# togheppi/pytorch-super-resolution-model-collection

Measured on AMD Instinct MI355X. Metric: ESPCN x4 LR->HR images/sec (infer), higher is better.
Workload: dtype f32 storage/accumulate; fp32-faithful products on the fp16 matrix cores: operands scaled by exact powers of two, split into two fp16 planes, 3 MFMAs per product (f16x3, ~3e-7 rms vs fp64, like fp32 MFMA); 1 GPU; c2: ESPCN x4 inference, 256x256 LR, batch 64 per GPU, fp32, random-init N(0,0.02); parallelism=replicas x1 (no collective)

## Files before the change

pytorch_super_resolution_model_collection_amd/csrc/conv_pair.hip:

```cpp
#include "conv_bfw.h"

namespace srk {

namespace {

constexpr int PR_TH = 8, PR_TW = 16, PR_HW = 18;
constexpr int PR_NSLOTPIX = 6 * PR_HW, PR_NPIXP = PR_NSLOTPIX + 2;
constexpr int PR_NKEEP = 2 * PR_HW, PR_KP = PR_NKEEP + 2;
constexpr int PR_XR = 14, PR_XC = 23, PR_XP = 24;
constexpr int PR_NSLOT = 3, PR_NKBUF = 3;
constexpr int PR_WL2 = 9 * 2 * 256;
constexpr int PR_HBUF = 4 * PR_NPIXP;
constexpr int PR_KBUF = 2 * 4 * PR_KP;
constexpr int PR_PLANE = PR_NSLOT * PR_HBUF + PR_NKBUF * PR_KBUF;
constexpr int PR_XPQ = PR_XR * PR_XP * 16;
constexpr int PR_XT = PR_XPQ + 32;
constexpr int PR_XBUF = PR_XT + PR_XR * PR_XP * 8;
constexpr unsigned long long PR_FPIX = 0xfdb9eca875316420ull;
constexpr unsigned PR_AMAX_CAP = 1u << 14;
constexpr int PR_ARRIVE = 1, PR_DEPART = 2;
constexpr int PR_XLD = 24;
constexpr int PR_W1P = 2 * 2 * 8 * 64;
constexpr int PR_W1P_FLOATS = 144;
constexpr size_t PR_W1P_BYTES = (size_t)PR_W1P * 16 + PR_W1P_FLOATS * 4;
constexpr size_t PR_LDS = (size_t)PR_WL2 * 16 + (size_t)2 * PR_PLANE * 16 + (size_t)2 * PR_XBUF + 64;
static_assert(PR_LDS <= 160 * 1024, "k_espcn_pair: LDS");

__device__ unsigned g_pair_timeouts = 0;
__device__ unsigned g_pair_scans = 0;

typedef unsigned v4u_t __attribute__((ext_vector_type(4)));

struct PairParams {
  const float* x;
  const uint4* w1p;
  const float* b1;
  const uint4* wq2;
  const float* w2_descale;
  const float* b2;
  float* y;
  float* x_amax;
  float* y_amax;
  size_t xn;
  int amax_mode;
  int N, H, W, OH, OW, tiles_y, img_tiles, ntiles;
  unsigned x_img_bytes, y_bytes;
};

__device__ __forceinline__ float pr_slice_absmax(const float* __restrict__ x, size_t lo, size_t hi, size_t n, bool tail,
                                                 int t, int nt) {
  const f32x4* x4 = reinterpret_cast<const f32x4*>(x);
  float m = 0.f;
  for (size_t base = lo; base < hi; base += (size_t)nt * PR_XLD) {
    f32x4 v[PR_XLD];
#pragma unroll
    for (int k = 0; k < PR_XLD; ++k) {
      const size_t e = base + (size_t)t + (size_t)k * nt;
      v[k] = x4[e < hi ? e : hi - 1];
    }
#pragma unroll
    for (int k = 0; k < PR_XLD; ++k) m = abs_max4(m, v[k]);
  }
  if (tail) {
    const size_t e = (n & ~(size_t)3) + (size_t)t;
    if (t < 3 && e < n) m = fmaxf(m, fabsf(x[e]));
  }
  return m;
}

enum { PR_KTAP, PR_KROW, PR_KNONE };
struct PrKGroup {
  int kind, dy, dx;
};
__device__ __forceinline__ constexpr PrKGroup pr_kgroup(int ks, int kq) {
  if (ks < 5) return {PR_KTAP, ks, kq};
  if (ks == 5) return {PR_KTAP, (kq >> 1) + 2 * (kq & 1), 4};
  if (ks == 6) return kq == 0 ? PrKGroup{PR_KTAP, 4, 4} : (kq == 1 ? PrKGroup{PR_KNONE, 0, 0} : PrKGroup{PR_KROW, 2 * kq - 4, 0});
  return kq == 3 ? PrKGroup{PR_KNONE, 0, 0} : PrKGroup{PR_KROW, kq == 2 ? 4 : 2 * kq + 1, 0};
}

__global__ __launch_bounds__(128) void k_espcn_pair_prep(const float* __restrict__ w1, const float* __restrict__ b1,
                                                         uint4* __restrict__ out) {
  const int lane = threadIdx.x & 63, c1 = threadIdx.x >> 6;
  const int j = lane & 15, kq = lane >> 4;
  float wsum = 0.f, wmax = 0.f;
  {
    const float* wc = w1 + lane * 75;
    for (int i = 0; i < 75; ++i) {
      const float a = fabsf(wc[i]);
      wsum += a;
      wmax = fmaxf(wmax, a);
    }
  }
  const float wm = wave_max(wmax);
  const float sw1 = exp2i(amax_scale_exp(wm));
#pragma unroll
  for (int nf = 0; nf < 2; ++nf) {
    const int co = c1 * 32 + nf * 16 + j;
#pragma unroll
    for (int ks = 0; ks < 8; ++ks) {
      const PrKGroup g = pr_kgroup(ks, kq);
      float f[8];
#pragma unroll
      for (int e = 0; e < 8; ++e) {
        const bool tap = g.kind == PR_KTAP;
        const bool on = tap || (g.kind == PR_KROW && e < 5);
        const int ci = tap ? (e < 6 ? e % 3 : e - 6) : 2, dx = tap ? g.dx : (e < 5 ? e : 0);
        f[e] = on ? w1[((co * 3 + ci) * 5 + g.dy) * 5 + dx] : 0.f;
      }
      uint4 pl[2];
      split8h(f, sw1, pl);
      out[((c1 * 2 + nf) * 8 + ks) * 64 + lane] = g.kind == PR_KTAP ? make_uint4(pl[0].x, pl[0].y, pl[0].z, pl[1].w) : pl[1];
    }
  }
  if (c1 == 0) {
    float* t = reinterpret_cast<float*>(out + PR_W1P);
    t[lane] = wsum;
    t[64 + lane] = fabsf(b1[lane]);
    if (lane == 0) t[128] = wm;
  }
}

__global__ __launch_bounds__(512, 1) void k_espcn_pair(PairParams B) {
  extern __shared__ __attribute__((aligned(16))) uint4 smem4[];
  uint4* wl2 = smem4;
  uint4* ring = smem4 + PR_WL2;
  uint4* keep = ring + PR_NSLOT * PR_HBUF;
  unsigned char* xin_all = reinterpret_cast<unsigned char*>(ring + 2 * PR_PLANE);
  lds_cnt_t* cnt = (lds_cnt_t*)(xin_all + 2 * PR_XBUF);
  const int tid = threadIdx.x, lane = tid & 63, wave = tid >> 6;
  const int grp = wave >> 2, gw = wave & 3, lt = tid & 255;
  const int j = lane & 15, kq = lane >> 4;
  unsigned char* xin = xin_all + grp * PR_XBUF;

  const float* w1t = reinterpret_cast<const float*>(B.w1p + PR_W1P);
  const int nblk = gridDim.x;
  float xmax = 0.f;
  if (tid < 14) cnt[tid] = 0u;
  if (B.amax_mode) {
    float* red = reinterpret_cast<float*>(xin_all);
    const size_t n4 = B.xn >> 2;
    const float m = wave_max(pr_slice_absmax(B.x, (size_t)blockIdx.x * n4 / nblk, (size_t)(blockIdx.x + 1) * n4 / nblk, B.xn,
                                             blockIdx.x == 0, tid, 512));
    if (lane == 0) red[wave] = m;
    __syncthreads();
    if (tid == 0) {
      float b = red[0];
#pragma unroll
      for (int i = 1; i < 8; ++i) b = fmaxf(b, red[i]);
      const unsigned was = atomicMax(reinterpret_cast<unsigned*>(B.x_amax + (blockIdx.x & 15) * 16), __float_as_uint(b));
      asm volatile("s_waitcnt vmcnt(0)" ::"v"(was) : "memory");
      __hip_atomic_fetch_add(reinterpret_cast<unsigned*>(B.x_amax) + PR_ARRIVE, 1u, __ATOMIC_RELAXED, __HIP_MEMORY_SCOPE_AGENT);
    }
  } else {
    xmax = amax_read(B.x_amax);
  }

  {
    static_assert(PR_WL2 == 9 * 512, "k_espcn_pair: filter copy");
    v4u_t wv[9];
#pragma unroll
    for (int i = 0; i < 9; ++i) wv[i] = *reinterpret_cast<const v4u_t*>(B.wq2 + tid + 512 * i);
#pragma unroll
    for (int i = 0; i < 9; ++i) *reinterpret_cast<v4u_t*>(wl2 + tid + 512 * i) = wv[i];
  }

  const int c1 = gw >> 1, mh = gw & 1;
  const int mhu = __builtin_amdgcn_readfirstlane(mh), rhu = __builtin_amdgcn_readfirstlane(gw >> 1);
  uint4 w1f[2][8];
#pragma unroll
  for (int nf = 0; nf < 2; ++nf)
#pragma unroll
    for (int ks = 0; ks < 8; ++ks) w1f[nf][ks] = B.w1p[((c1 * 2 + nf) * 8 + ks) * 64 + lane];
  const float wsum = w1t[lane], babs = w1t[64 + lane];
  const int jp = (int)((PR_FPIX >> (4 * j)) & 15);
  int mpix[5], moff[5], tpix[2], toff[2];
#pragma unroll
  for (int m = 0; m < 5; ++m) {
    mpix[m] = 16 * (m < 4 ? 4 * mh + m : 8) + jp;
    const int p = PR_NKEEP + mpix[m];
    moff[m] = (p / PR_HW) * PR_XP + p % PR_HW + kq;
  }
#pragma unroll
  for (int m = 0; m < 2; ++m) {
    tpix[m] = 16 * (2 * mh + m) + jp;
    const int p = tpix[m] < PR_NKEEP ? tpix[m] : PR_NKEEP - 1;
    toff[m] = (p / PR_HW) * PR_XP + p % PR_HW + kq;
  }
  const int k5 = pr_kgroup(5, kq).dy * PR_XP + 4 - kq;
  int kmul[2], kadd[2], kd[2];
#pragma unroll
  for (int s = 0; s < 2; ++s) {
    const PrKGroup own = pr_kgroup(6 + s, kq), g = own.kind == PR_KNONE ? pr_kgroup(6 + s, kq - 1) : own;
    kmul[s] = g.kind == PR_KTAP ? 16 : 8;
    kd[s] = g.kind == PR_KTAP ? 8 : 32;
    asm volatile("" : "+v"(kd[s]));
    kadd[s] = g.kind == PR_KTAP ? 16 * (g.dy * PR_XP + g.dx - kq) : PR_XT + 8 * (g.dy * PR_XP - kq);
  }
  const int wr_slot = (kq >> 1) * PR_NPIXP * 16 + (kq & 1) * 8, wr_keep = (c1 * 4 + (kq >> 1)) * PR_KP * 16 + (kq & 1) * 8;

  const int rh = gw >> 1, nf2 = gw & 1;
  const int pj = j < 4 ? 2 * j : (j < 12 ? 2 * j - 7 : 2 * j - 16);
  const int lane_b = (4 * rh - 2) * PR_HW + pj + kq * PR_NPIXP;
  const int lane_k = pj + kq * PR_KP;
  const int lane_a = kq * 32 + nf2 * 16 + j;
  float b2v[4];
#pragma unroll
  for (int e = 0; e < 4; ++e) b2v[e] = B.b2[nf2 * 16 + 4 * kq + e];

  const int xcd = blockIdx.x & 7;
  int first, count;
  {
    const int lb = xcd * (nblk >> 3) + (xcd < (nblk & 7) ? xcd : (nblk & 7)) + (blockIdx.x >> 3);
    const int per = B.ntiles / nblk, rem = B.ntiles - per * nblk;
    first = lb * per + (lb < rem ? lb : rem);
    count = per + (lb < rem ? 1 : 0);
  }
  count = __builtin_amdgcn_readfirstlane(count);

  const __amdgpu_buffer_rsrc_t yr = buffer_rsrc(B.y, B.y_bytes);
  const unsigned HW_ = (unsigned)(B.H * B.W);
  float xv[2][3];
  auto xload = [&](int i) {
    const bool valid = i < count;
    const int t = first + (valid ? i : 0);
    const int n = t / B.img_tiles, rem = t - n * B.img_tiles;
    const int tx = rem / B.tiles_y, ty = rem - tx * B.tiles_y;
    const __amdgpu_buffer_rsrc_t xr = buffer_rsrc(B.x + (size_t)n * 3 * HW_, B.x_img_bytes);
#pragma unroll
    for (int s = 0; s < 2; ++s) {
      const int q = lt + 256 * s, qy = q / PR_XC, qx = q - qy * PR_XC;
      const bool ok = valid && q < PR_XR * PR_XC;
      const unsigned o = ok ? 4u * (unsigned)((ty * PR_TH + qy) * B.W + tx * PR_TW + qx) : 0x80000000u;
#pragma unroll
      for (int c = 0; c < 3; ++c)
        xv[s][c] = __builtin_bit_cast(float, __builtin_amdgcn_raw_buffer_load_b32(xr, (int)(o + (ok ? 4u * c * HW_ : 0u)), 0, 0));
    }
  };
  auto l1_frags = [&](auto nm, const int* off, f32x4 (*a)[2]) {
    constexpr int NM = decltype(nm)::value;
#pragma unroll
    for (int m = 0; m < NM; ++m) a[m][0] = a[m][1] = (f32x4){0.f, 0.f, 0.f, 0.f};
#pragma unroll
    for (int ks = 0; ks < 8; ++ks) {
#pragma unroll
      for (int m = 0; m < NM; ++m) {
        uint4 xc;
        if (ks < 6) {
          xc = *reinterpret_cast<const uint4*>(xin + 16 * (off[m] + (ks < 5 ? ks * PR_XP : k5)));
        } else {
          const int pa = __mul24(off[m], kmul[ks & 1]) + kadd[ks & 1];
          const uint2 ca = *reinterpret_cast<const uint2*>(xin + pa), cb = *reinterpret_cast<const uint2*>(xin + pa + kd[ks & 1]);
          xc = make_uint4(ca.x, ca.y, cb.x, cb.y);
        }
#pragma unroll
        for (int nf = 0; nf < 2; ++nf) a[m][nf] = mfma16h(w1f[nf][ks], xc, a[m][nf]);
      }
    }
  };
  bool dead = false;
  float amax = 0.f;
  xload(grp);
  if (B.amax_mode && wave == 0) {
    unsigned* ctr = reinterpret_cast<unsigned*>(B.x_amax);
    bool late = B.amax_mode == 2;
    if (!late) {
      unsigned spins = 0;
      while ((int)((unsigned)__builtin_amdgcn_readfirstlane((int)__hip_atomic_load(ctr + PR_ARRIVE, __ATOMIC_RELAXED,
                                                                                   __HIP_MEMORY_SCOPE_AGENT)) -
                   (unsigned)nblk) < 0) {
        __builtin_amdgcn_s_sleep(16);
        if (++spins > PR_AMAX_CAP) {
          late = true;
          break;
        }
      }
    }
    asm volatile("" ::: "memory");
    const float sv = wave_max(__hip_atomic_load(B.x_amax + (lane & 15) * 16, __ATOMIC_RELAXED, __HIP_MEMORY_SCOPE_AGENT));
    if (lane == 0) {
      cnt[14] = __float_as_uint(sv);
      cnt[15] = late ? 1u : 0u;
      const unsigned d = __hip_atomic_fetch_add(ctr + PR_DEPART, 1u, __ATOMIC_RELAXED, __HIP_MEMORY_SCOPE_AGENT);
      if (d + 1u == (unsigned)nblk) {
        __hip_atomic_store(ctr + PR_ARRIVE, 0u, __ATOMIC_RELAXED, __HIP_MEMORY_SCOPE_AGENT);
        __hip_atomic_store(ctr + PR_DEPART, 0u, __ATOMIC_RELAXED, __HIP_MEMORY_SCOPE_AGENT);
      }
    }
  }
  __syncthreads();
  if (B.amax_mode) {
    xmax = __uint_as_float(lds_cnt_peek(cnt + 14));
    if (lds_cnt_peek(cnt + 15)) {
      float* red = reinterpret_cast<float*>(xin_all);
      const float m = wave_max(pr_slice_absmax(B.x, 0, B.xn >> 2, B.xn, true, tid, 512));
      if (lane == 0) red[wave] = m;
      __syncthreads();
#pragma unroll
      for (int i = 0; i < 8; ++i) xmax = fmaxf(xmax, red[i]);
      xmax = __uint_as_float((unsigned)__builtin_amdgcn_readfirstlane((int)__float_as_uint(xmax)));
      __syncthreads();
      if (tid == 0) atomicAdd(&g_pair_scans, 1u);
    }
  }
  for (int i = tid; i < 2 * PR_XBUF / 16; i += 512) reinterpret_cast<uint4*>(xin_all)[i] = make_uint4(0u, 0u, 0u, 0u);
  __syncthreads();
  const int kx = amax_scale_exp(xmax);
  const float bnd = wave_max(fabsf(babs) + wsum * xmax);
  const int kw1 = amax_scale_exp(w1t[128]);
  const int km = amax_scale_exp(bnd);
  const float sx1 = exp2i(kx), sxm = exp2i(km);
  const float dsc1 = exp2i(-kx) * exp2i(-kw1);
  const float dsc2 = exp2i(-km) * B.w2_descale[0];

  unsigned own = 0;
  unsigned kseq = 0;
  int typrev = 0;
  for (int i = grp; i < count; i += 2, ++own) {
    const int t = first + i;
    const int n = t / B.img_tiles, rem = t - n * B.img_tiles;
    const int tx = rem / B.tiles_y, ty = rem - tx * B.tiles_y;
    const bool fresh = i == 0 || ty == 0;
    const bool hand = i + 1 < count && ty + 1 < B.tiles_y;
    kseq = i == grp ? (grp == 0 ? 1u : 2u + (ty == 0 ? 1u : 0u))
                    : kseq + 2u + (typrev + 1 == B.tiles_y ? 1u : 0u) + (ty == 0 ? 1u : 0u);
    typrev = ty;
    const unsigned kb = kseq % PR_NKBUF, ku = kseq / PR_NKBUF, tb = (kseq - 1u) % PR_NKBUF, tu = (kseq - 1u) / PR_NKBUF;
#pragma unroll
    for (int s = 0; s < 2; ++s) {
      const int q = lt + 256 * s;
      if (q < PR_XR * PR_XC) {
        const int qy = q / PR_XC, qx = q - qy * PR_XC;
        unsigned h01, m01, h2, m2;
        split2h(xv[s][0], xv[s][1], sx1, h01, m01);
        split2h(xv[s][2], 0.f, sx1, h2, m2);
        *reinterpret_cast<uint4*>(xin + 16 * (qy * PR_XP + qx)) = make_uint4(h01, h2 | (m01 << 16), (m01 >> 16) | (m2 << 16), h01);
        unsigned short* tq = reinterpret_cast<unsigned short*>(xin + PR_XT) + 4 * (qy * PR_XP + qx);
#pragma unroll
        for (int k = 0; k < 4; ++k) tq[-3 * k] = (unsigned short)h2;
      }
    }
    lds_cnt_signal(cnt + 6 + grp);
    xload(i + 2);
    lds_cnt_wait(cnt + 6 + grp, 4u * (own + 1), dead);

    float b1v[2][4];
#pragma unroll
    for (int nf = 0; nf < 2; ++nf)
#pragma unroll
      for (int e = 0; e < 4; ++e) b1v[nf][e] = B.b1[c1 * 32 + nf * 16 + 4 * kq + e];
    auto l1_store = [&](const f32x4 (&a)[2], unsigned char* base, int pix, int pitch) {
#pragma unroll
      for (int nf = 0; nf < 2; ++nf) {
        float v[4];
#pragma unroll
        for (int e = 0; e < 4; ++e) v[e] = fmaxf(__builtin_fmaf(a[nf][e], dsc1, b1v[nf][e]), 0.f);
        unsigned h01, m01, h23, m23;
        split2h(v[0], v[1], sxm, h01, m01);
        split2h(v[2], v[3], sxm, h23, m23);
        *reinterpret_cast<uint2*>(base + ((2 * nf) * pitch + pix) * 16) = make_uint2(h01, h23);
        *reinterpret_cast<uint2*>(base + (PR_PLANE + (2 * nf) * pitch + pix) * 16) = make_uint2(m01, m23);
      }
    };
    auto l1_tile = [&](auto nm) {
      constexpr int NM = decltype(nm)::value;
      f32x4 a1[NM][2];
      l1_frags(nm, moff, a1);
      const unsigned st = 2u * (unsigned)i + c1, slot = st % PR_NSLOT, use = st / PR_NSLOT;
      unsigned char* hb = reinterpret_cast<unsigned char*>(ring + slot * PR_HBUF) + wr_slot;
      lds_cnt_wait(cnt + 3 + slot, 4u * use, dead);
#pragma unroll
      for (int m = 0; m < NM; ++m)
        if (mpix[m] < PR_NSLOTPIX) l1_store(a1[m], hb, mpix[m], PR_NPIXP);
      lds_cnt_signal(cnt + slot);
      unsigned char* kp = reinterpret_cast<unsigned char*>(keep + kb * PR_KBUF) + wr_keep;
      lds_cnt_wait(cnt + 11 + kb, 8u * ku, dead);
#pragma unroll
      for (int m = 2; m < NM; ++m)
        if (mpix[m] >= PR_NSLOTPIX) l1_store(a1[m], kp, mpix[m] - PR_NSLOTPIX, PR_KP);
      lds_cnt_signal(cnt + 8 + kb);
    };
    const int vr = B.OH - ty * PR_TH;
    if (mhu == 1 && vr <= 3) {
      const unsigned st = 2u * (unsigned)i + c1, slot = st % PR_NSLOT, use = st / PR_NSLOT;
      lds_cnt_wait(cnt + 3 + slot, 4u * use, dead);
      lds_cnt_signal(cnt + slot);
      lds_cnt_wait(cnt + 11 + kb, 8u * ku, dead);
      lds_cnt_signal(cnt + 8 + kb);
    } else if (mh == (int)(own & 1)) {
      l1_tile(std::integral_constant<int, 5>{});
    } else {
      l1_tile(std::integral_constant<int, 4>{});
    }
    if (fresh) {
      f32x4 at[2][2];
      l1_frags(std::integral_constant<int, 2>{}, toff, at);
      unsigned char* kp = reinterpret_cast<unsigned char*>(keep + tb * PR_KBUF) + wr_keep;
      lds_cnt_wait(cnt + 11 + tb, 8u * tu, dead);
#pragma unroll
      for (int m = 0; m < 2; ++m)
        if (tpix[m] < PR_NKEEP) l1_store(at[m], kp, tpix[m], PR_KP);
      lds_cnt_signal(cnt + 8 + tb);
    }

    lds_cnt_wait(cnt + 8 + (rh == 0 ? tb : kb), 4u * ((rh == 0 ? tu : ku) + 1u), dead);
    if (rhu == 1 && vr <= 4) {
#pragma unroll
      for (int cc = 0; cc < 2; ++cc) {
        const unsigned st = 2u * (unsigned)i + cc, slot = st % PR_NSLOT, use = st / PR_NSLOT;
        lds_cnt_wait(cnt + slot, 2u * (use + 1), dead);
        lds_cnt_signal(cnt + 3 + slot);
      }
      lds_cnt_signal(cnt + 11 + tb, fresh ? 2u : 1u);
      lds_cnt_signal(cnt + 11 + kb, hand ? 1u : 2u);
    } else {
      f32x4 acc[4];
#pragma unroll
      for (int r = 0; r < 4; ++r) acc[r] = (f32x4){0.f, 0.f, 0.f, 0.f};
#pragma unroll
      for (int cc = 0; cc < 2; ++cc) {
        const unsigned st = 2u * (unsigned)i + cc, slot = st % PR_NSLOT, use = st / PR_NSLOT;
        lds_cnt_wait(cnt + slot, 2u * (use + 1), dead);
        const uint4* hb = ring + slot * PR_HBUF + lane_b;
        const uint4* kr = keep + (rh == 0 ? tb : kb) * PR_KBUF + cc * 4 * PR_KP + lane_k - (rh == 0 ? 0 : 4 * PR_HW);
        const uint4* pa = rh == 0 ? kr : hb;
        const uint4* pc = rh == 0 ? hb : kr;
#pragma unroll
        for (int v = 0; v < 3; ++v) {
          uint4 fa[3][2];
#pragma unroll
          for (int u = 0; u < 3; ++u) {
            fa[u][0] = wl2[((u * 3 + v) * 2 + cc) * 256 + lane_a];
            fa[u][1] = wl2[((u * 3 + v) * 2 + cc) * 256 + 128 + lane_a];
          }
#pragma unroll
          for (int R = 0; R < 6; ++R) {
            const uint4* px = R < 2 ? pa : (R < 4 ? hb : pc);
            const uint4 xh = px[R * PR_HW + v], xm = px[R * PR_HW + v + PR_PLANE];
#pragma unroll
            for (int u = 0; u < 3; ++u) {
              const int r = R - u;
              if (r >= 0 && r < 4) {
                acc[r] = mfma16h(fa[u][0], xm, acc[r]);
                acc[r] = mfma16h(fa[u][1], xh, acc[r]);
                acc[r] = mfma16h(fa[u][0], xh, acc[r]);
              }
            }
          }
        }
        lds_cnt_signal(cnt + 3 + slot);
      }
      lds_cnt_signal(cnt + 11 + tb, fresh ? 2u : 1u);
      lds_cnt_signal(cnt + 11 + kb, hand ? 1u : 2u);
      const int oc = tx * PR_TW + pj;
#pragma unroll
      for (int r = 0; r < 4; ++r) {
        const int orow = ty * PR_TH + 4 * rh + r;
        const bool ok = oc < B.OW && orow < B.OH;
        f32x4 v;
#pragma unroll
        for (int e = 0; e < 4; ++e) v[e] = fmaxf(__builtin_fmaf(acc[r][e], dsc2, b2v[e]), 0.f);
        if (ok) amax = fmaxf(amax, fmaxf(fmaxf(v[0], v[1]), fmaxf(v[2], v[3])));
        const unsigned o = ok ? 4u * (unsigned)(((n * B.OH + orow) * B.OW + oc) * 32 + nf2 * 16 + 4 * kq) : 0x80000000u;
        __builtin_amdgcn_raw_buffer_store_b128(__builtin_bit_cast(v4u_t, v), yr, (int)o, 0, 0);
      }
    }
  }
  if (B.y_amax) amax_commit(B.y_amax, amax, blockIdx.x + wave, amax_peek(B.y_amax, blockIdx.x + wave));
  if (dead && lane == 0) atomicAdd(&g_pair_timeouts, 1u);
}

}

int espcn_pair_launch(int N, int H, int W, const float* x, const void* w1p, const float* b1, const void* wp2,
                      const float* b2, float* y, float* x_amax, int amax_mode, float* y_amax, bool force, hipStream_t s) {
  if (N < 1 || H < 7 || W < 7 || !x_amax) return -1;
  const int OH = H - 6, OW = W - 6;
  const int tiles_y = (OH + PR_TH - 1) / PR_TH, tiles_x = (OW + PR_TW - 1) / PR_TW;
  const long ntiles = (long)N * tiles_y * tiles_x;
  const size_t x_img = (size_t)3 * H * W * 4, y_bytes = (size_t)N * OH * OW * 32 * 4;
  if (ntiles >= (1L << 29) || x_img >= (1ull << 31) || y_bytes >= (1ull << 31)) return -1;
  if (!force) {
    if ((double)OH * OW < 0.85 * (double)tiles_y * tiles_x * (PR_TH * PR_TW)) return -1;
    if (ntiles < 4L * kNumCU) return -1;
  }
  const size_t elems = (size_t)9 * 64 * 32;
  const char* prepared = reinterpret_cast<const char*>(wp2) + bf3_prepared_offset(elems);
  const char* fsec = prepared + f16_section_offset(64, 32, 9);
  PairParams B{};
  B.x = x; B.w1p = reinterpret_cast<const uint4*>(w1p); B.b1 = b1; B.b2 = b2; B.y = y; B.x_amax = x_amax; B.y_amax = y_amax;
  B.xn = (size_t)N * 3 * H * W;
  B.amax_mode = amax_mode;
  B.wq2 = reinterpret_cast<const uint4*>(fsec);
  B.w2_descale = reinterpret_cast<const float*>(fsec + bf3_main_bytes(64, 32, 9));
  B.N = N; B.H = H; B.W = W; B.OH = OH; B.OW = OW; B.tiles_y = tiles_y; B.img_tiles = tiles_x * tiles_y;
  B.ntiles = (int)ntiles;
  B.x_img_bytes = (unsigned)x_img;
  B.y_bytes = (unsigned)y_bytes;
  int grid = kNumCU;
  if (grid > ntiles) grid = (int)ntiles;
  note_amax_written(y_amax != nullptr);
  note_kernel("k_espcn_pair");
  launch_lds<&k_espcn_pair>(dim3(grid), dim3(512), PR_LDS, s, B);
  return check_launch("espcn_pair");
}

int pair_ring_timeouts(int reset) {
  unsigned v = 0;
  if (hipMemcpyFromSymbol(&v, HIP_SYMBOL(g_pair_timeouts), sizeof(v)) != hipSuccess) {
    (void)hipGetLastError();
    return -1;
  }
  if (reset && v) {
    const unsigned z = 0;
    (void)hipMemcpyToSymbol(HIP_SYMBOL(g_pair_timeouts), &z, sizeof(z));
  }
  return (int)v;
}

int pair_scans(int reset) {
  unsigned v = 0;
  if (hipMemcpyFromSymbol(&v, HIP_SYMBOL(g_pair_scans), sizeof(v)) != hipSuccess) {
    (void)hipGetLastError();
    return -1;
  }
  if (reset && v) {
    const unsigned z = 0;
    (void)hipMemcpyToSymbol(HIP_SYMBOL(g_pair_scans), &z, sizeof(z));
  }
  return (int)v;
}

int espcn_pair_prepare(const float* w1, const float* b1, void* out, hipStream_t s) {
  hipLaunchKernelGGL(k_espcn_pair_prep, dim3(1), dim3(128), 0, s, w1, b1, reinterpret_cast<uint4*>(out));
  return check_launch("espcn_pair_prepare");
}
size_t espcn_pair_prepared_bytes() { return PR_W1P_BYTES; }

}

extern "C" size_t srk_espcn_pair_prepared_bytes(void) { return srk::espcn_pair_prepared_bytes(); }

extern "C" int srk_espcn_pair_prepare(const float* w1, const float* b1, void* w1_prepared, void* stream) {
  SRK_REQUIRE(w1 && b1 && w1_prepared, "espcn_pair_prepare: null pointer");
  SRK_REQUIRE((uintptr_t)w1_prepared % 16 == 0, "espcn_pair_prepare: w1_prepared must be 16-byte aligned");
  return srk::espcn_pair_prepare(w1, b1, w1_prepared, (hipStream_t)stream);
}

extern "C" int srk_espcn_pair_scans(int reset) { return srk::pair_scans(reset); }

extern "C" int srk_espcn_pair_forward(int N, int H, int W, const float* x, const void* w1_prepared, const float* b1,
                                      const float* w2_packed_fwd, const float* b2, float* y, float* x_amax,
                                      int x_amax_compute, float* y_amax, int force, void* stream) {
  if (!x || !w1_prepared || !b1 || !w2_packed_fwd || !b2 || !y || !x_amax) return SRK_ERR_UNSUPPORTED;
  if (((uintptr_t)x | (uintptr_t)y | (uintptr_t)w1_prepared) % 16 != 0) return SRK_ERR_UNSUPPORTED;
  const int mode = x_amax_compute ? ((force & 2) ? 2 : 1) : 0;
  const int rc = srk::espcn_pair_launch(N, H, W, x, w1_prepared, b1, w2_packed_fwd, b2, y, x_amax, mode, y_amax,
                                        (force & 1) != 0, (hipStream_t)stream);
  return rc == -1 ? SRK_ERR_UNSUPPORTED : rc;
}
```

Before: 76280 images/s.

## Software-pipeline LDS operand loads with MFMAs and overlap next-slot wait in conv pair

Restructures the inner MFMA loop of the paired conv kernel into a fully unrolled schedule. Weight (A) and pixel (B) fragments are prefetched one to two steps ahead in rotating registers, with sched_barriers pinning the interleaving. The wait on the second ring slot is split into an early relaxed peek plus a late spin. The slot-release signal also moves earlier, before the last MFMAs of each slot, so producers can refill sooner. This aims to hide LDS latency and synchronization stalls behind matrix work, at the cost of more register pressure and a rigid instruction schedule.

Result: faster. 77720 images/s, median of 6 (+1.9%).

```diff
diff --git a/pytorch_super_resolution_model_collection_amd/csrc/conv_pair.hip b/pytorch_super_resolution_model_collection_amd/csrc/conv_pair.hip
--- a/pytorch_super_resolution_model_collection_amd/csrc/conv_pair.hip
+++ b/pytorch_super_resolution_model_collection_amd/csrc/conv_pair.hip
@@ -417,39 +417,83 @@
       f32x4 acc[4];
 #pragma unroll
       for (int r = 0; r < 4; ++r) acc[r] = (f32x4){0.f, 0.f, 0.f, 0.f};
+      uint4 fa[3][2], fb[3][2];
+      const uint4 *spa[2], *shb[2], *spc[2];
+      unsigned sslot[2], suse[2];
 #pragma unroll
       for (int cc = 0; cc < 2; ++cc) {
-        const unsigned st = 2u * (unsigned)i + cc, slot = st % PR_NSLOT, use = st / PR_NSLOT;
-        lds_cnt_wait(cnt + slot, 2u * (use + 1), dead);
-        const uint4* hb = ring + slot * PR_HBUF + lane_b;
+        const unsigned st = 2u * (unsigned)i + cc;
+        sslot[cc] = st % PR_NSLOT;
+        suse[cc] = st / PR_NSLOT;
+        shb[cc] = ring + sslot[cc] * PR_HBUF + lane_b;
         const uint4* kr = keep + (rh == 0 ? tb : kb) * PR_KBUF + cc * 4 * PR_KP + lane_k - (rh == 0 ? 0 : 4 * PR_HW);
-        const uint4* pa = rh == 0 ? kr : hb;
-        const uint4* pc = rh == 0 ? hb : kr;
-#pragma unroll
-        for (int v = 0; v < 3; ++v) {
-          uint4 fa[3][2];
-#pragma unroll
-          for (int u = 0; u < 3; ++u) {
-            fa[u][0] = wl2[((u * 3 + v) * 2 + cc) * 256 + lane_a];
-            fa[u][1] = wl2[((u * 3 + v) * 2 + cc) * 256 + 128 + lane_a];
-          }
-#pragma unroll
-          for (int R = 0; R < 6; ++R) {
-            const uint4* px = R < 2 ? pa : (R < 4 ? hb : pc);
-            const uint4 xh = px[R * PR_HW + v], xm = px[R * PR_HW + v + PR_PLANE];
-#pragma unroll
-            for (int u = 0; u < 3; ++u) {
-              const int r = R - u;
-              if (r >= 0 && r < 4) {
-                acc[r] = mfma16h(fa[u][0], xm, acc[r]);
-                acc[r] = mfma16h(fa[u][1], xh, acc[r]);
-                acc[r] = mfma16h(fa[u][0], xh, acc[r]);
+        spa[cc] = rh == 0 ? kr : shb[cc];
+        spc[cc] = rh == 0 ? shb[cc] : kr;
+      }
+      auto ldA = [&](auto uc, auto vc, auto ccc) {
+        constexpr int u = decltype(uc)::value, v = decltype(vc)::value, cc = decltype(ccc)::value;
+        fa[u][0] = wl2[((u * 3 + v) * 2 + cc) * 256 + lane_a];
+        fa[u][1] = wl2[((u * 3 + v) * 2 + cc) * 256 + 128 + lane_a];
+      };
+      auto ldB = [&](auto ccc, auto sc) {
+        constexpr int cc = decltype(ccc)::value, s = decltype(sc)::value, v = s / 6, R = s - 6 * v;
+        const uint4* px = R < 2 ? spa[cc] : (R < 4 ? shb[cc] : spc[cc]);
+        fb[s % 3][0] = px[R * PR_HW + v];
+        fb[s % 3][1] = px[R * PR_HW + v + PR_PLANE];
+      };
+      using I0 = std::integral_constant<int, 0>;
+      using I1 = std::integral_constant<int, 1>;
+      using I2 = std::integral_constant<int, 2>;
+      lds_cnt_wait(cnt + sslot[0], 2u * (suse[0] + 1), dead);
+      ldA(I0{}, I0{}, I0{});
+      ldB(I0{}, I0{});
+      ldA(I1{}, I0{}, I0{});
+      ldB(I0{}, I1{});
+      srk_static_for<0, 2>([&](auto ccc) {
+        constexpr int cc = decltype(ccc)::value;
+        unsigned peek_v = 0;
+        srk_static_for<0, 18>([&](auto sc) {
+          constexpr int s = decltype(sc)::value, v = s / 6, R = s - 6 * v;
+          constexpr int u_lo = R - 3 > 0 ? R - 3 : 0, u_hi = R < 2 ? R : 2;
+          srk_static_for<u_lo, u_hi + 1>([&](auto uc) {
+            constexpr int u = decltype(uc)::value, r = R - u;
+            acc[r] = mfma16h(fa[u][0], fb[s % 3][1], acc[r]);
+            acc[r] = mfma16h(fa[u][1], fb[s % 3][0], acc[r]);
+            acc[r] = mfma16h(fa[u][0], fb[s % 3][0], acc[r]);
+            __builtin_amdgcn_sched_barrier(0);
+            if constexpr (u == u_lo) {
+              if constexpr (cc == 0 && s == 16) {
+                if (!dead) {
+                  unsigned seen = (unsigned)__builtin_amdgcn_readfirstlane((int)peek_v), spins = 0;
+                  while ((int)(seen - 2u * (suse[1] + 1)) < 0) {
+                    __builtin_amdgcn_s_sleep(1);
+                    seen = lds_cnt_peek(cnt + sslot[1]);
+                    if (++spins > kLdsCntSpinCap) {
+                      dead = true;
+                      break;
+                    }
+                  }
+                }
+                asm volatile("" ::: "memory");
+              }
+              if constexpr (s + 2 < 18) ldB(ccc, std::integral_constant<int, s + 2>{});
+              else if constexpr (cc == 0) ldB(I1{}, std::integral_constant<int, s + 2 - 18>{});
+              if constexpr (cc == 0 && s == 8)
+                peek_v = __hip_atomic_load(cnt + sslot[1], __ATOMIC_RELAXED, __HIP_MEMORY_SCOPE_WORKGROUP);
+              if constexpr (s == 15) lds_cnt_signal(cnt + 3 + sslot[cc]);
+              __builtin_amdgcn_sched_barrier(0);
+              if constexpr (R == 0) {
+                ldA(I2{}, std::integral_constant<int, v>{}, ccc);
+                __builtin_amdgcn_sched_barrier(0);
+              } else if constexpr (R >= 4) {
+                if constexpr (v < 2) ldA(std::integral_constant<int, R - 4>{}, std::integral_constant<int, v + 1>{}, ccc);
+                else if constexpr (cc == 0) ldA(std::integral_constant<int, R - 4>{}, I0{}, I1{});
+                __builtin_amdgcn_sched_barrier(0);
               }
             }
-          }
-        }
-        lds_cnt_signal(cnt + 3 + slot);
-      }
+          });
+        });
+      });
       lds_cnt_signal(cnt + 11 + tb, fresh ? 2u : 1u);
       lds_cnt_signal(cnt + 11 + kb, hand ? 1u : 2u);
       const int oc = tx * PR_TW + pj;
```
